# moxime/joint-vae

Hardware: AMD Instinct MI355X
Metric: training_images_per_sec (higher is better)
Workload: dtype f32

## Files before the change

### include/jvae_hip.h

```cpp
#ifndef JVAE_HIP_H
#define JVAE_HIP_H

#include <stddef.h>

#ifdef __cplusplus
extern "C" {
#endif

const char* jvae_version(void);

int jvae_gemm_f32(int M, int N, int K, int batch,
                  const float* A, long sAm, long sAk, long sAb,
                  const float* B, long sBk, long sBn, long sBb,
                  float* C, long sCm, long sCn, long sCb,
                  const float* bias, int bias_mode, int flags, int splitk, void* stream);

int jvae_splitk_fold_f32(const float* part, const float* bias, float* y, int S, long MN, int N, int relu, int accumulate,
                         void* stream);

size_t jvae_conv2d_workspace_bytes(int N, int Cin, int H, int W, int Cout, int KH, int KW, int S, int P, int OP,
                                   int transposed);
int jvae_conv2d_set_split_bf16(int mode);
int jvae_conv2d_set_split_shape16(int on);
int jvae_conv2d_out_shape(int H, int W, int KH, int KW, int S, int P, int OP, int transposed, int* OH, int* OW);
int jvae_conv2d_route(int dir, int layout, int bias, int stats, int y_f32, int aff_kind,
                      int N, int Cin, int H, int W, int Cout, int KH, int KW, int S, int P, int OP, int transposed,
                      int* kernel, int* swap, size_t* ws_bytes, int* splits, int* aff_ok);
const char* jvae_conv2d_kernel_name(int kernel);
int jvae_conv2d_fwd_f32(const float* x, const float* w, const float* bias, float* y,
                        int N, int Cin, int H, int W, int Cout, int KH, int KW, int S, int P, int OP, int transposed,
                        void* ws, size_t ws_bytes, void* stream);
int jvae_conv2d_stats_splits(int N, int Cin, int H, int W, int Cout, int KH, int KW, int S, int P, int OP, int transposed);
int jvae_conv2d_fwd_stats_f32(const float* x, const float* w, const float* bias, float* y, float* stats, int* nsplit,
                              int N, int Cin, int H, int W, int Cout, int KH, int KW, int S, int P, int OP, int transposed,
                              void* ws, size_t ws_bytes, void* stream);
int jvae_conv2d_dgrad_f32(const float* dy, const float* w, float* dx,
                          int N, int Cin, int H, int W, int Cout, int KH, int KW, int S, int P, int OP, int transposed,
                          void* ws, size_t ws_bytes, void* stream);
int jvae_conv2d_wgrad_f32(const float* x, const float* dy, float* dw, float* dbias, int accumulate,
                          int N, int Cin, int H, int W, int Cout, int KH, int KW, int S, int P, int OP, int transposed,
                          void* ws, size_t ws_bytes, void* stream);

int jvae_pack_cache_configure(void* buf, size_t bytes);
int jvae_pack_cache_begin(void* stream, long long owner, const void* const* weights, int n);
int jvae_pack_cache_end(void);
int jvae_pack_cache_pin(void);
int jvae_pack_cache_reset(void);
int jvae_pack_cache_stats(int* entries, long long* hits, long long* misses, long long* refreshes);

size_t jvae_channel_sum_workspace_bytes(int C);
int jvae_channel_sum_f32(const float* t, float* out, int N, int C, int P, int accumulate, void* ws, size_t ws_bytes,
                         void* stream);

size_t jvae_bn_workspace_bytes(int C);
int jvae_bn_plan(int N, int C, int P, int* nsplit, int* nchunk);
int jvae_image_range(int N, int parts, int j, int* nb, int* ne);
// ... 295 lines not shown
```

### joint-vae_amd/csrc/conv_api.hip

```cpp
#include "common.h"
#include "jvae_internal.h"
#include "conv_dispatch.h"

namespace {

inline ConvRoute route(const ConvGeom& g, int transposed, ConvDir dir, CallFlags f = {}) {
    return jvae_conv_route(g, transposed, dir, CONV_F32, f);
}

bool affine_ok(const ConvGeom& g, int transposed, ConvDir other, const ConvRoute& r) {
    return r.aff_ok && route(g, transposed, other, {false, false, false, 1}).aff_ok;
}

int fwd_f32(const float* x, const float* w, const float* bias, float* y, float* stats, int* nsplit, const InAff* aff,
            int N, int Cin, int H, int W, int Cout, int KH, int KW, int S, int P, int OP, int transposed,
            void* ws, size_t ws_bytes, void* stream) {
    ConvGeom g; int oh, ow;
    if (nsplit) *nsplit = 0;
    if (!jvae_make_geom(N, Cin, H, W, Cout, KH, KW, S, P, OP, transposed, &g, &oh, &ow)) return JVAE_EINVAL;
    const ConvRoute r = route(g, transposed, CONV_FWD, {bias != nullptr, stats != nullptr, false, jvae_aff_kind(aff)});
    if (aff && !affine_ok(g, transposed, CONV_WGRAD, r)) return JVAE_ENOTSUP;
    if (N == 0) return 0;
    if (jvae_ws_short(r, ws, ws_bytes)) return JVAE_EWORKSPACE;
    return jvae_conv_run_fwd(r, g, x, w, bias, y, (float*)ws, ws_bytes, (hipStream_t)stream, stats, nsplit, aff);
// ... 39 lines not shown
    if (!jvae_make_geom(N, Cin, H, W, Cout, KH, KW, S, P, OP, transposed, &g, &oh, &ow)) return 0;
    return jvae_conv_ws(g, transposed);
}

int jvae_conv2d_route(int dir, int layout, int bias, int stats, int y_f32, int aff_kind,
                      int N, int Cin, int H, int W, int Cout, int KH, int KW, int S, int P, int OP, int transposed,
                      int* kernel, int* swap, size_t* ws_bytes, int* splits, int* aff_ok) {
    ConvGeom g; int oh, ow;
    if (dir != CONV_FWD && dir != CONV_DGRAD && dir != CONV_WGRAD) return JVAE_EINVAL;
    if ((layout != CONV_F32 && layout != CONV_B8) || aff_kind < 0 || aff_kind > 2) return JVAE_EINVAL;
    if (!jvae_make_geom(N, Cin, H, W, Cout, KH, KW, S, P, OP, transposed, &g, &oh, &ow)) return JVAE_EINVAL;
    const ConvRoute r = jvae_conv_route(g, transposed, (ConvDir)dir, (ConvLayout)layout,
                                        {bias != 0, stats != 0, y_f32 != 0, aff_kind});
    if (kernel) *kernel = (int)r.k;
    if (swap) *swap = r.swap ? 1 : 0;
    if (ws_bytes) *ws_bytes = r.ws;
    if (splits) *splits = r.splits;
    if (aff_ok) *aff_ok = r.aff_ok ? 1 : 0;
    return 0;
}

const char* jvae_conv2d_kernel_name(int kernel) {
    switch (kernel) {
#define JVAE_CK_NAME(k) case k: return #k;
        JVAE_CK_NAME(CK_NONE) JVAE_CK_NAME(CK_GENERIC) JVAE_CK_NAME(CK_POINT) JVAE_CK_NAME(CK_SMALLCO)
        JVAE_CK_NAME(CK_SMALLCI) JVAE_CK_NAME(CK_FWD5) JVAE_CK_NAME(CK_FWD5_X3) JVAE_CK_NAME(CK_T2) JVAE_CK_NAME(CK_T2_X3)
        JVAE_CK_NAME(CK_WG5) JVAE_CK_NAME(CK_WG5_X3) JVAE_CK_NAME(CK_B8) JVAE_CK_NAME(CK_T2_B8) JVAE_CK_NAME(CK_WG_B8)
        JVAE_CK_NAME(CK_WG_B8X) JVAE_CK_NAME(CK_SMALLCO_DG)
#undef JVAE_CK_NAME
        default: return nullptr;
    }
}

int jvae_conv2d_out_shape(int H, int W, int KH, int KW, int S, int P, int OP, int transposed, int* OH, int* OW) {
    ConvGeom g;
    if (!OH || !OW) return JVAE_EINVAL;
    return jvae_make_geom(1, 1, H, W, 1, KH, KW, S, P, OP, transposed, &g, OH, OW) ? 0 : JVAE_EINVAL;
}

int jvae_conv2d_fwd_f32(const float* x, const float* w, const float* bias, float* y,
                        int N, int Cin, int H, int W, int Cout, int KH, int KW, int S, int P, int OP, int transposed,
                        void* ws, size_t ws_bytes, void* stream) {
    if (!w || (N > 0 && (!x || !y))) return JVAE_EINVAL;
    return fwd_f32(x, w, bias, y, nullptr, nullptr, nullptr, N, Cin, H, W, Cout, KH, KW, S, P, OP, transposed, ws, ws_bytes,
                   stream);
}

int jvae_conv2d_stats_splits(int N, int Cin, int H, int W, int Cout, int KH, int KW, int S, int P, int OP, int transposed) {
    ConvGeom g; int oh, ow;
    if (!jvae_make_geom(N, Cin, H, W, Cout, KH, KW, S, P, OP, transposed, &g, &oh, &ow)) return 0;
    return route(g, transposed, CONV_FWD, {false, true, false, 0}).splits;
}

int jvae_conv2d_fwd_stats_f32(const float* x, const float* w, const float* bias, float* y, float* stats, int* nsplit,
                              int N, int Cin, int H, int W, int Cout, int KH, int KW, int S, int P, int OP, int transposed,
                              void* ws, size_t ws_bytes, void* stream) {
    if (!w || !nsplit || (N > 0 && (!x || !y))) return JVAE_EINVAL;
    return fwd_f32(x, w, bias, y, stats, nsplit, nullptr, N, Cin, H, W, Cout, KH, KW, S, P, OP, transposed, ws, ws_bytes, stream);
}

int jvae_conv2d_affine_ok(int N, int Cin, int H, int W, int Cout, int KH, int KW, int S, int P, int OP, int transposed) {
    ConvGeom g; int oh, ow;
    if (!jvae_make_geom(N, Cin, H, W, Cout, KH, KW, S, P, OP, transposed, &g, &oh, &ow)) return 0;
    return affine_ok(g, transposed, CONV_WGRAD, route(g, transposed, CONV_FWD, {false, false, false, 1})) ? 1 : 0;
}

// ... 47 lines not shown
```

### joint-vae_amd/csrc/conv_dispatch.h

```cpp
#pragma once
#include "common.h"
#include "jvae_internal.h"

size_t jvae_conv_generic_ws(const ConvGeom& g);
int jvae_fold_fwd(const ConvGeom& g, const float* xb, const float* w, const float* bias, float* ys,
                  float* ws, size_t ws_bytes, hipStream_t st);
int jvae_fold_bwd(const ConvGeom& g, const float* ys, const float* w, const float* bias, float* xb,
                  float* ws, size_t ws_bytes, hipStream_t st);
int jvae_fold_wgrad(const ConvGeom& g, const float* xb, const float* ys, float* dw,
                    float* ws, size_t ws_bytes, hipStream_t st);
size_t jvae_channel_sum_ws_bytes(int C);
int jvae_channel_sum(const float* t, float* out, int N, int C, int P, int accumulate, float* ws, size_t ws_bytes,
                     hipStream_t st);

bool jvae_conv5_fwd_ok(int Cin, int H, int W, int Cout, int OH, int OW, int S, int P);
size_t jvae_conv5_pack_floats(int Cin, int Cout);
int jvae_conv5_fwd(const float* in, const float* w, int swap, int flip, const float* bias, float* out,
                   int N, int Cin, int H, int W, int Cout, int OW, int S, int P, float* ws, hipStream_t st,
                   float* stats = nullptr, int* nsplit = nullptr, const InAff* aff = nullptr);
int jvae_conv5_fwd_max_splits(int N, int OW);

int jvae_conv5_pack(const float* w, float* wp, int C, int O, int swap, int flip, hipStream_t st);

bool jvae_conv5_x3_ok(int Cin, int H, int W, int Cout, int OH, int OW, int S, int P);
// ... 3 lines not shown
bool jvae_conv5_x3_enabled();
int jvae_conv5_x3_wpack(const float* w, float* ws, int C, int O, int swap, int flip, hipStream_t st);
bool jvae_convt2_x3_ok(int N, int C, int WS, int O);
int jvae_convt2_x3(const float* in, const float* w, const float* bias, float* out, int N, int C, int WS, int O, float* ws,
                   hipStream_t st, float* stats = nullptr, int* nsplit = nullptr, const InAff* aff = nullptr);
int jvae_conv5_x3_fwd(const float* in, const float* w, int swap, int flip, const float* bias, float* out,
                      int N, int Cin, int H, int W, int Cout, int OW, int S, int P, float* ws, hipStream_t st,
                      float* stats = nullptr, int* nsplit = nullptr, const InAff* aff = nullptr);

bool jvae_convt2_ok(int C, int HS, int WS, int O, int HB, int WB, int KH, int KW, int S, int P);
int jvae_convt2(const float* in, const float* wpacked, const float* bias, float* out, int N, int C, int WS, int O,
                hipStream_t st, float* stats = nullptr, int* nsplit = nullptr, const InAff* aff = nullptr);

bool jvae_conv5_smallco_ok(int Cin, int H, int W, int Cout, int KH, int KW, int S, int P);
int jvae_conv5_smallco(const float* in, const float* w, const float* bias, float* out, int N, int Cin, int W, int Cout,
                       hipStream_t st, const InAff* aff = nullptr);
int jvae_conv5_smallco_dgrad(const float* dy, const float* w, float* dx, int N, int Cy, int W, int Cx, hipStream_t st);

bool jvae_conv5_smallci_ok(int Cin, int H, int W, int Cout, int OW, int S, int P, bool dgrad_role);
int jvae_conv5_smallci(const float* in, const float* w, int swap, int flip, const float* bias, float* out,
                       int N, int Cin, int W, int Cout, float* ws, hipStream_t st, float* stats = nullptr, int* nsplit = nullptr);

bool jvae_conv5_wgrad_ok(int Ca, int HS, int WS, int Cb, int HB, int WB, int S, int P);
size_t jvae_conv5_wgrad_ws_floats(int N, int Ca, int Cb, int S, int WS);
int jvae_conv5_wgrad(const float* ps, const float* q, float* dw, int accumulate, int swapflip,
                     int N, int Ca, int WS, int Cb, int S, int P, float* ws, hipStream_t st,
                     const InAff* aff_p = nullptr, const InAff* aff_q = nullptr);

bool jvae_conv5_wgrad_x3_ok(int Ca, int HS, int WS, int Cb, int HB, int WB, int S, int P);
size_t jvae_conv5_wgrad_x3_ws_floats(int N, int Ca, int Cb, int S);
int jvae_conv5_wgrad_x3(const float* ps, const float* q, float* dw, int accumulate, int swapflip,
                        int N, int Ca, int WS, int Cb, int S, int P, float* ws, hipStream_t st,
                        const InAff* aff_p = nullptr, const InAff* aff_q = nullptr);

bool jvae_make_geom(int N, int Cin, int H, int W, int Cout, int KH, int KW, int S, int P, int OP, int transposed,
                    ConvGeom* g, int* OH, int* OW);

enum ConvDir { CONV_FWD = 1, CONV_DGRAD = 2, CONV_WGRAD = 4 };
enum ConvLayout { CONV_F32, CONV_B8 };
enum ConvKernel {
    CK_NONE,
    CK_GENERIC, CK_POINT,
    CK_SMALLCO, CK_SMALLCI, CK_FWD5, CK_FWD5_X3, CK_T2, CK_T2_X3, CK_WG5, CK_WG5_X3,
    CK_B8, CK_T2_B8, CK_WG_B8, CK_WG_B8X,
    CK_SMALLCO_DG,
};
struct CallFlags {
    bool bias, stats;
    bool y_f32;
    int aff;
};
struct ConvRoute {
    ConvKernel k;
    bool swap;
    int S, P;
    size_t ws;
    int splits;
    bool aff_ok;
};
ConvRoute jvae_conv_route(const ConvGeom& g, int transposed, ConvDir dir, ConvLayout layout, CallFlags f);
inline int jvae_aff_kind(const InAff* aff) { return !aff ? 0 : (aff->relu == JVAE_ACT_LEAKY ? 2 : 1); }
inline bool jvae_ws_short(const ConvRoute& r, const void* ws, size_t ws_bytes) { return r.ws && (!ws || ws_bytes < r.ws); }
template <class T>
inline void jvae_wgrad_operands(const ConvRoute& r, int transposed, T* x, T* dy, const InAff* aff, T** ps, T** q,
                                const InAff** aff_p, const InAff** aff_q) {
    const bool p_is_x = r.swap != (transposed != 0);
    *ps = p_is_x ? x : dy;
    *q = p_is_x ? dy : x;
    *aff_p = p_is_x ? aff : nullptr;
    *aff_q = p_is_x ? nullptr : aff;
}

size_t jvae_conv_ws(const ConvGeom& g, int transposed);
int jvae_conv_run_fwd(const ConvRoute& r, const ConvGeom& g, const float* in, const float* w, const float* bias, float* out,
                      float* ws, size_t ws_bytes, hipStream_t st, float* stats = nullptr, int* nsplit = nullptr,
                      const InAff* aff = nullptr);
int jvae_conv_run_wgrad(const ConvRoute& r, const ConvGeom& g, int transposed, const float* x, const float* dy, float* dw,
                        float* ws, size_t ws_bytes, hipStream_t st, const InAff* aff = nullptr);
```

### joint-vae_amd/csrc/conv_dispatch.hip

```cpp
#include "common.h"
#include "conv_dispatch.h"
#include "conv_b8.h"
#include "pack_elems.h"

namespace {

inline bool is5(const ConvGeom& g) { return g.KH == 5 && g.KW == 5; }
inline bool is3p1(const ConvGeom& g) { return g.KH == 3 && g.KW == 3 && g.P == 1; }
inline size_t max_sz(size_t a, size_t b) { return a > b ? a : b; }

inline bool point_input(const ConvGeom& g) {
    return g.Hs == 1 && g.Ws == 1 && g.P == 0 && g.S == 1 && g.Hb == g.KH && g.Wb == g.KW;
}
inline int point_wgrad_pieces(const ConvGeom& g) {
    const int want = (int)(1024 / ((long)cdiv(g.Cs, 64) * cdiv(g.Cb * g.KH * g.KW, 64)));
    return want < 1 ? 1 : (want > 8 ? 8 : want);
}

struct FwdOp { int Ci, H, W, Co, OH, OW; };
inline FwdOp fwd_op(const ConvGeom& g, bool small_in) {
    return small_in ? FwdOp{g.Cs, g.Hs, g.Ws, g.Cb, g.Hb, g.Wb} : FwdOp{g.Cb, g.Hb, g.Wb, g.Cs, g.Hs, g.Ws};
}
struct WgOp { int Ca, HS, WS, Cb, HB, WB; };
inline WgOp wg_op(const ConvGeom& g, bool swap) {
// ... 73 lines not shown
}

inline const float* packed_f32(const float* w, float* ws, int C, int O, int swap, int flip, hipStream_t st) {
    return (const float*)jvae_packed(JVAE_PACK_F32, w, C, O, swap, flip, ws,
                                     [&](void* dst) { return jvae_conv5_pack(w, (float*)dst, C, O, swap, flip, st); });
}

}

bool jvae_make_geom(int N, int Cin, int H, int W, int Cout, int KH, int KW, int S, int P, int OP, int transposed,
                    ConvGeom* g, int* OH, int* OW) {
    if (N < 0 || Cin <= 0 || Cout <= 0 || H <= 0 || W <= 0 || KH <= 0 || KW <= 0 || S <= 0 || P < 0 || OP < 0)
        return false;
    g->N = N; g->KH = KH; g->KW = KW; g->S = S; g->P = P;
    if (!transposed) {
        if (OP != 0) return false;
        *OH = (H + 2 * P - KH) / S + 1;
        *OW = (W + 2 * P - KW) / S + 1;
        g->Cb = Cin; g->Hb = H; g->Wb = W;
        g->Cs = Cout; g->Hs = *OH; g->Ws = *OW;
    } else {
        if (OP >= S && OP != 0) return false;
        *OH = (H - 1) * S - 2 * P + KH + OP;
        *OW = (W - 1) * S - 2 * P + KW + OP;
        g->Cs = Cin; g->Hs = H; g->Ws = W;
        g->Cb = Cout; g->Hb = *OH; g->Wb = *OW;
    }
    return *OH > 0 && *OW > 0;
}

ConvRoute jvae_conv_route(const ConvGeom& g, int transposed, ConvDir dir, ConvLayout layout, CallFlags f) {
    if (dir == CONV_WGRAD) return wgrad_route(g, transposed, layout == CONV_B8, f);
    return fwd_route(g, transposed, dir, layout == CONV_B8, f);
}

size_t jvae_conv_ws(const ConvGeom& g, int transposed) {
    size_t a = max_sz(jvae_conv_generic_ws(g), jvae_channel_sum_ws_bytes(g.Cb > g.Cs ? g.Cb : g.Cs));
    for (ConvDir d : {CONV_FWD, CONV_DGRAD, CONV_WGRAD}) a = max_sz(a, jvae_conv_route(g, transposed, d, CONV_F32, {}).ws);
    if (is5(g)) a = max_sz(a, 4 * jvae_conv5_pack_floats(g.Cb, g.Cs));
    if (transposed && point_input(g)) a = max_sz(a, 4 * (size_t)8 * g.Cs * g.Cb * g.KH * g.KW);
    return a;
}

int jvae_conv_run_fwd(const ConvRoute& r, const ConvGeom& g, const float* in, const float* w, const float* bias, float* out,
                      float* ws, size_t ws_bytes, hipStream_t st, float* stats, int* nsplit, const InAff* aff) {
    const FwdOp o = fwd_op(g, r.swap);
    const int sw = r.swap ? 1 : 0;
    switch (r.k) {
        case CK_SMALLCO: return jvae_conv5_smallco(in, w, bias, out, g.N, g.Cb, g.Wb, g.Cs, st, aff);
        case CK_SMALLCO_DG: return jvae_conv5_smallco_dgrad(in, w, out, g.N, g.Cs, g.Wb, g.Cb, st);
        case CK_SMALLCI: return jvae_conv5_smallci(in, w, sw, sw, bias, out, g.N, o.Ci, o.W, o.Co, ws, st, stats, nsplit);
        case CK_FWD5_X3:
            return jvae_conv5_x3_fwd(in, w, sw, sw, bias, out, g.N, o.Ci, o.H, o.W, o.Co, o.OW, r.S, r.P, ws, st, stats, nsplit, aff);
        case CK_FWD5:
            return jvae_conv5_fwd(in, w, sw, sw, bias, out, g.N, o.Ci, o.H, o.W, o.Co, o.OW, r.S, r.P, ws, st, stats, nsplit, aff);
        case CK_T2_X3: return jvae_convt2_x3(in, w, bias, out, g.N, g.Cs, g.Ws, g.Cb, ws, st, stats, nsplit, aff);
        case CK_T2: {
            const float* wp = packed_f32(w, ws, g.Cs, g.Cb, 1, 0, st);
            if (!wp) return JVAE_EINVAL;
            return jvae_convt2(in, wp, bias, out, g.N, g.Cs, g.Ws, g.Cb, st, stats, nsplit, aff);
        }
        case CK_POINT: {
            const int cols = g.Cb * g.KH * g.KW;
            if (r.swap)
                return jvae_gemm_launch_ex(g.N, cols, g.Cs, 1, in, g.Cs, 1, 0, w, cols, 1, 0, out, cols, 1, 0,
                                           bias, bias ? 1 : 0, g.KH * g.KW, 0, 1, st);
// ... 41 lines not shown
```

### joint-vae_amd/csrc/conv_wgrad_x3.hip

```cpp
#include <stdlib.h>
#include "common.h"
#include "jvae_internal.h"
#include "conv_dispatch.h"
#include "conv_x3.h"

namespace {

typedef x3_bf16x8 bf16x8;
typedef __bf16 bf16x4 __attribute__((ext_vector_type(4)));
typedef x3_u32x4 u32x4;
typedef x3_f32x2 f32x2;
typedef __attribute__((address_space(3))) bf16x4 lds_bf16x4;

struct WgX3P {
    const void* ps;
    const void* q;
    float* slab;
    int N, Ca, Cb, P, G;
    InAff aff_p, aff_q;
};

template <int S, int WS, int MODE, int NPL = 3>
struct WgX3Geom {
    static constexpr int HS = WS;
// ... 437 lines not shown
                else if (MODE == 2) { b = cbq0 * 8 + c16; tap = wave + 4 * (2 * t + cb); }
                else if (MODE == 3) { b = j & 3; tap = tile * 8 + (j >> 2); }
                else { b = j & 7; tap = tile * 4 + (j >> 3); }
                if (b >= p.Cb || tap > 24) continue;
#pragma unroll
                for (int rb = 0; rb < 2; ++rb)
#pragma unroll
                    for (int r = 0; r < 4; ++r) {
                        const int a = a0 + rb * 16 + g16 * 4 + r;
                        if (a < p.Ca) slab[((long)a * 25 + tap) * p.Cb + b] = acc16[t][rb][cb][r];
                    }
            }
        }
        return;
    }
#pragma unroll
    for (int t = 0; t < G::NBT; ++t) {
        const int tile = wave + 4 * t;
        if (tile >= G::NTILE) continue;
        int b, tap;
        if (MODE == 0) { b = cbq0 * 8 + l31; tap = tile; }
        else if (MODE == 2) { b = cbq0 * 8 + (l31 & 15); tap = tile * 2 + (l31 >> 4); }
        else if (MODE == 3) { b = l31 & 3; tap = tile * 8 + (l31 >> 2); }
        else { b = l31 & 7; tap = tile * 4 + (l31 >> 3); }
        if (b >= p.Cb || tap > 24) continue;
#pragma unroll
        for (int r = 0; r < 16; ++r) {
            const int a = a0 + (r & 3) + 8 * (r >> 2) + 4 * half;
            if (a < p.Ca) slab[((long)a * 25 + tap) * p.Cb + b] = acc[t][r];
        }
    }
}

template <int S, int WS, int MODE, int NPL = 3>
int launch_wgx3(const WgX3P& p, hipStream_t st) {
    using G = WgX3Geom<S, WS, MODE, NPL>;
    static_assert(G::LDS_BYTES + 2048 <= 80 * 1024, "two workgroups per CU must fit the 160 KB LDS");
    dim3 grid(p.G, (p.Ca + 31) / 32, (p.Cb + 8 * G::NCBQ - 1) / (8 * G::NCBQ));
    if (MODE == 1 || MODE == 3) grid.z = 1;
    const bool aff = p.aff_p.sc || p.aff_q.sc;
    const bool leaky = (p.aff_p.sc && p.aff_p.relu == JVAE_ACT_LEAKY) || (p.aff_q.sc && p.aff_q.relu == JVAE_ACT_LEAKY);
    if constexpr (NPL == 1) {
        static bool attr1 = false;
        if (!attr1) {
            const void* fns[2] = {reinterpret_cast<const void*>(&conv5_wgrad_x3_kernel<S, WS, MODE, 0, true, 1>),
                                  reinterpret_cast<const void*>(&conv5_wgrad_x3_kernel<S, WS, MODE, 1, true, 1>)};
            for (const void* f : fns) {
                hipError_t e = hipFuncSetAttribute(f, hipFuncAttributeMaxDynamicSharedMemorySize, G::LDS_BYTES);
                if (e != hipSuccess) return (int)e;
            }
            attr1 = true;
        }
        if (aff) hipLaunchKernelGGL((conv5_wgrad_x3_kernel<S, WS, MODE, 1, true, 1>), grid, dim3(256), G::LDS_BYTES, st, p);
        else hipLaunchKernelGGL((conv5_wgrad_x3_kernel<S, WS, MODE, 0, true, 1>), grid, dim3(256), G::LDS_BYTES, st, p);
        JVAE_LAUNCH_CHECK();
        return 0;
    } else {
    static bool attr_set = false;
    auto kernel = [](auto A) { return &conv5_wgrad_x3_kernel<S, WS, MODE, decltype(A)::value, true>; };
    if (const int rc = jvae_aff_lds_attr(attr_set, G::LDS_BYTES, kernel)) return rc;
    jvae_with_aff(leaky ? 2 : (aff ? 1 : 0), [&](auto A) { hipLaunchKernelGGL(kernel(A), grid, dim3(256), G::LDS_BYTES, st, p); });
    JVAE_LAUNCH_CHECK();
    return 0;
    }
}

inline int x3_mode(int S, int Cb) { return Cb <= 4 ? 3 : (Cb <= 8 ? 1 : (S == 2 ? 2 : 0)); }

int slab_count_x3(int N, int Ca, int Cb, int S) {
    const int mode = x3_mode(S, Cb);
    const int gz = (mode == 1 || mode == 3) ? 1 : (mode == 2 ? (Cb + 15) / 16 : (Cb + 31) / 32);
    const int per = ((Ca + 31) / 32) * gz;
    int target = 512 / per;
    if (target < 1) target = 1;
    int imgs = (N + target - 1) / target;
    if (imgs < 1) imgs = 1;
    return (N + imgs - 1) / imgs;
}

}

bool jvae_conv5_wgrad_x3_ok(int Ca, int HS, int WS, int Cb, int HB, int WB, int S, int P) {
    if (!jvae_conv5_x3_enabled()) return false;
    if (S != 1 && S != 2) return false;
    if (HS != WS || HB != WB || WB != WS * S) return false;
    if (WS != 8 && WS != 16 && WS != 32) return false;
    if (P < 0 || P > 4 || Ca < 16 || Cb < 1) return false;
    if (P + WB > (WS - 1) * S + 5) return false;
    return true;
}

size_t jvae_conv5_wgrad_x3_ws_floats(int N, int Ca, int Cb, int S) { return (size_t)slab_count_x3(N, Ca, Cb, S) * Ca * Cb * 25; }

int jvae_conv5_wgrad_x3(const float* ps, const float* q, float* dw, int accumulate, int swapflip,
                        int N, int Ca, int WS, int Cb, int S, int P, float* ws, hipStream_t st,
                        const InAff* aff_p, const InAff* aff_q) {
    const InAff none{nullptr, nullptr, 0};
    WgX3P p{ps, q, ws, N, Ca, Cb, P, slab_count_x3(N, Ca, Cb, S), aff_p ? *aff_p : none, aff_q ? *aff_q : none};
    int rc = JVAE_ENOTSUP;
    const int mode = x3_mode(S, Cb);
#define WGX3_CASE(S_, WS_, M_) case WS_: rc = launch_wgx3<S_, WS_, M_>(p, st); break;
    if (mode == 3 && S == 1) {
        switch (WS) { WGX3_CASE(1, 8, 3) WGX3_CASE(1, 16, 3) WGX3_CASE(1, 32, 3) }
    } else if (mode == 3) {
        switch (WS) { WGX3_CASE(2, 8, 3) WGX3_CASE(2, 16, 3) WGX3_CASE(2, 32, 3) }
    } else if (mode == 1 && S == 1) {
        switch (WS) { WGX3_CASE(1, 8, 1) WGX3_CASE(1, 16, 1) WGX3_CASE(1, 32, 1) }
    } else if (mode == 1) {
        switch (WS) { WGX3_CASE(2, 8, 1) WGX3_CASE(2, 16, 1) WGX3_CASE(2, 32, 1) }
    } else if (mode == 0) {
        switch (WS) { WGX3_CASE(1, 8, 0) WGX3_CASE(1, 16, 0) WGX3_CASE(1, 32, 0) }
    } else {
        switch (WS) { WGX3_CASE(2, 8, 2) WGX3_CASE(2, 16, 2) WGX3_CASE(2, 32, 2) }
    }
#undef WGX3_CASE
    if (rc) return rc;
    return jvae_wgrad_slab_reduce(ws, dw, p.G, Ca, Cb, accumulate, swapflip, st, 1);
}

bool jvae_conv5_wgrad_b8x_ok(int Ca, int HS, int WS, int Cb, int HB, int WB, int S, int P) {
    if (S != 1 && S != 2) return false;
    if (HS != WS || HB != WB || WB != WS * S) return false;
    if (WS != 8 && WS != 16 && WS != 32 && !(WS == 64 && S == 1)) return false;
    if (P < 0 || P > 4 || Ca < 16 || Cb < 1) return false;
    if (P + WB > (WS - 1) * S + 5) return false;
    return true;
}

size_t jvae_conv5_wgrad_b8x_ws_floats(int N, int Ca, int Cb, int S) { return (size_t)slab_count_x3(N, Ca, Cb, S) * Ca * Cb * 25; }

int jvae_conv5_wgrad_b8x(const void* ps, const void* q, float* dw, int accumulate, int swapflip,
                         int N, int Ca, int WS, int Cb, int S, int P, float* ws, hipStream_t st,
                         const InAff* aff_p, const InAff* aff_q) {
    const InAff none{nullptr, nullptr, 0};
    WgX3P p{ps, q, ws, N, Ca, Cb, P, slab_count_x3(N, Ca, Cb, S), aff_p ? *aff_p : none, aff_q ? *aff_q : none};
// ... 21 lines not shown
```

### joint-vae_amd/jvae_hip/lib.py

```python
import ctypes
import os
from ctypes import c_char_p, c_float, c_int, c_long, c_longlong, c_size_t, c_void_p, POINTER

import torch

_HERE = os.path.dirname(os.path.abspath(__file__))
LIB_PATH = os.environ.get('JVAE_HIP_LIB') or os.path.join(_HERE, 'libjvae_hip.so')

_lib = None

P = c_void_p
_SIGS = {
    'jvae_version': (c_char_p, []),
    'jvae_gemm_f32': (c_int, [c_int] * 4 + [P, c_long, c_long, c_long] * 3 + [P, c_int, c_int, c_int, P]),
    'jvae_splitk_fold_f32': (c_int, [P, P, P, c_int, c_long, c_int, c_int, c_int, P]),
    'jvae_conv2d_workspace_bytes': (c_size_t, [c_int] * 11),
    'jvae_conv2d_set_split_bf16': (c_int, [c_int]),
    'jvae_conv2d_set_split_shape16': (c_int, [c_int]),
    'jvae_conv2d_out_shape': (c_int, [c_int] * 8 + [POINTER(c_int), POINTER(c_int)]),
    'jvae_conv2d_route': (c_int, [c_int] * 17 + [POINTER(c_int), POINTER(c_int), POINTER(c_size_t), POINTER(c_int), POINTER(c_int)]),
    'jvae_conv2d_kernel_name': (c_char_p, [c_int]),
    'jvae_conv2d_fwd_f32': (c_int, [P, P, P, P] + [c_int] * 11 + [P, c_size_t, P]),
    'jvae_conv2d_stats_splits': (c_int, [c_int] * 11),
    'jvae_conv2d_fwd_stats_f32': (c_int, [P, P, P, P, P, POINTER(c_int)] + [c_int] * 11 + [P, c_size_t, P]),
    'jvae_conv2d_dgrad_f32': (c_int, [P, P, P] + [c_int] * 11 + [P, c_size_t, P]),
    'jvae_conv2d_wgrad_f32': (c_int, [P, P, P, P, c_int] + [c_int] * 11 + [P, c_size_t, P]),
    'jvae_b8_pack_f32': (c_int, [P, P, c_int, c_int, c_long, P]),
    'jvae_b8_unpack_f32': (c_int, [P, P, c_int, c_int, c_long, c_int, P]),
    'jvae_conv2d_native_b8': (c_int, [c_int] * 11),
    'jvae_conv2d_workspace_bytes_b8': (c_size_t, [c_int] * 11),
    'jvae_conv2d_stats_splits_b8': (c_int, [c_int] * 11),
    'jvae_conv2d_fwd_b8': (c_int, [P, P, P, P, c_int, P, POINTER(c_int)] + [c_int] * 11 + [P, c_size_t, P]),
    'jvae_conv2d_dgrad_b8': (c_int, [P, P, P] + [c_int] * 11 + [P, c_size_t, P]),
    'jvae_conv2d_wgrad_b8': (c_int, [P, P, P, P, c_int] + [c_int] * 11 + [P, c_size_t, P]),
    'jvae_bn_workspace_bytes_b8': (c_size_t, [c_int]),
    'jvae_bn_plan_b8': (c_int, [c_int, c_int, c_long, POINTER(c_int), POINTER(c_int)]),
    'jvae_bn_fwd_b8': (c_int, [P] * 9 + [c_int, c_int, c_long, c_float, c_float, c_int, c_int, P, c_int, P, P, c_size_t, P]),
    'jvae_bn_bwd_b8': (c_int, [P] * 9 + [c_int, c_int, c_int, c_long, c_int, P, c_size_t, P]),
    'jvae_bn_finalize_b8': (c_int, [P] * 9 + [c_int, c_int, c_long, c_float, c_float, c_int, P, c_int, P, P, c_size_t, P]),
    'jvae_bn_sums_b8': (c_int, [P, P, P, c_int, c_int, c_long, P, c_size_t, P]),
    'jvae_bn_fwd_sync_b8': (c_int, [P] * 9 + [c_int, c_int, c_long, c_float, c_float, c_int, P, P, c_int, P, c_size_t, P]),
    'jvae_bn_bwd_sums_b8': (c_int, [P] * 7 + [c_int, c_int, c_long, c_int, P, c_size_t, P]),
    'jvae_bn_bwd_sync_b8': (c_int, [P] * 8 + [c_int, P, P, P, c_int, c_int, c_int, c_long, c_int, P, c_size_t, P]),
    'jvae_conv2d_affine_ok_b8': (c_int, [c_int] * 11),
    'jvae_conv2d_fwd_aff_b8': (c_int, [P, P, P, P, c_int, P, POINTER(c_int), P, P, c_int] + [c_int] * 11 + [P, c_size_t, P]),
    'jvae_conv2d_wgrad_aff_b8': (c_int, [P, P, P, P, c_int, P, P, c_int] + [c_int] * 11 + [P, c_size_t, P]),
    'jvae_relu_fwd_b8': (c_int, [P, P, c_long, P]),
    'jvae_relu_bwd_b8': (c_int, [P, P, P, c_long, P]),
    'jvae_bn_finalize_f32': (c_int, [P] * 10 + [c_int, c_int, c_int, c_float, c_float, c_int, P, c_int, P, P, c_size_t, P]),
    'jvae_conv2d_affine_ok': (c_int, [c_int] * 11),
    'jvae_conv2d_fwd_aff_f32': (c_int, [P, P, P, P, P, POINTER(c_int), P, P, c_int] + [c_int] * 11 + [P, c_size_t, P]),
# ... 216 lines not shown
```

### joint-vae_amd/jvae_hip/ops.py

```python
import collections
import contextlib
import ctypes
import math
from ctypes import byref, c_int, c_size_t

import numpy as np
import torch

from . import lib as L

RELU, SIGMOID, IDENT, LEAKY = 1, 2, 0, 3
BN_ACT = {IDENT: 0, RELU: 1, LEAKY: 2}
OVERLAP_WGRAD = True
ACT_KIND = {'relu': RELU, 'sigmoid': SIGMOID, 'linear': IDENT, 'leaky': LEAKY, None: IDENT}


def _c(t):
    return t if t.is_contiguous() else t.contiguous()


def _f32(t, what):
    if t.dtype != torch.float32:
        raise L.JvaeHipError(f'{what}: fp32 expected, got {t.dtype}')
    return t
# ... 169 lines not shown
    lib = L.load()
    N, _, H, W = x.shape
    geom = spec.geom(N, H, W)
    cap = _geom_query('jvae_conv2d_stats_splits', geom)
    if cap <= 0:
        return conv_fwd_raw(x, w, b, spec), None, 0
    oh, ow = spec.out_hw(H, W)
    y = torch.empty((N, spec.cout, oh, ow), device=x.device, dtype=torch.float32)
    stats = torch.empty((spec.cout * cap * 2,), device=x.device, dtype=torch.float32)
    ws, nb = _conv_ws(geom, x.device)
    ns = c_int(0)
    rc = lib.jvae_conv2d_fwd_stats_f32(L.ptr(x), L.ptr(w), L.ptr(b), L.ptr(y), L.ptr(stats), byref(ns), *geom,
                                       L.ptr(ws), nb, L.stream_ptr())
    L.check(rc, 'jvae_conv2d_fwd_stats_f32')
    return y, (stats if ns.value > 0 else None), ns.value


def conv_affine_ok(spec, N, H, W):
    return bool(_geom_query('jvae_conv2d_affine_ok', spec.geom(N, H, W)))


ConvRoute = collections.namedtuple('ConvRoute', 'kernel swap ws splits aff_ok')
ROUTE_DIR = {'fwd': 1, 'dgrad': 2, 'wgrad': 4}
ROUTE_LAYOUT = {'f32': 0, 'b8': 1}


def conv_route(spec, N, H, W, direction, layout='f32', bias=False, stats=False, y_f32=False, aff=0):
    lib = L.load()
    k, sw, ns, ok, ws = c_int(), c_int(), c_int(), c_int(), c_size_t()
    rc = lib.jvae_conv2d_route(ROUTE_DIR[direction], ROUTE_LAYOUT[layout], int(bias), int(stats), int(y_f32), int(aff),
                               *spec.geom(N, H, W), byref(k), byref(sw), byref(ws), byref(ns), byref(ok))
    L.check(rc, 'jvae_conv2d_route')
    return ConvRoute(lib.jvae_conv2d_kernel_name(k.value).decode(), bool(sw.value), ws.value, ns.value, bool(ok.value))


class LaunchProbe:

    def __init__(self, match):
        self.match, self.events, self.armed = match, [], False

    def times_ms(self):
        return [a.elapsed_time(b) for a, b in self.events]


FWD_AFF_PROBE = None


def conv_fwd_aff_raw(x, w, b, spec, aff, want_stats):
    lib = L.load()
    N, _, H, W = x.shape
    geom = spec.geom(N, H, W)
    oh, ow = spec.out_hw(H, W)
    y = torch.empty((N, spec.cout, oh, ow), device=x.device, dtype=torch.float32)
    stats, ns = None, c_int(0)
    if want_stats:
        cap = _geom_query('jvae_conv2d_stats_splits', geom)
        if cap > 0:
            stats = torch.empty((spec.cout * cap * 2,), device=x.device, dtype=torch.float32)
    ws, nb = _conv_ws(geom, x.device)
    probe = FWD_AFF_PROBE
    timed = probe is not None and probe.armed and probe.match(spec, N, H)
    if timed:
        ev = (torch.cuda.Event(enable_timing=True), torch.cuda.Event(enable_timing=True))
        ev[0].record()
    rc = lib.jvae_conv2d_fwd_aff_f32(L.ptr(x), L.ptr(w), L.ptr(b), L.ptr(y), L.ptr(stats), byref(ns),
                                     L.ptr(aff[0]), L.ptr(aff[1]), int(aff[2]), *geom, L.ptr(ws), nb, L.stream_ptr())
# ... 1691 lines not shown
```

Before: 144,000.

## Add K-packed bf16x3 MFMA weight-gradient kernel for 5x5 stride-1 small-Cb convs

Adds a new wgrad kernel for 5x5 stride-1 convolutions with at most three output-side channels. It packs the kernel-width taps and channels into the MFMA K dimension using shifted LDS copies of the q rows, instead of using the mode-3 layout that wastes MFMA lanes. Global loads for the next tile are overlapped with the MFMA loop, and the kernel is enabled by default through an env toggle. The cost is a more complex LDS layout, extra MFMAs on two waves to cover the fifth kernel row, and higher LDS use per workgroup.

```diff
diff --git a/include/jvae_hip.h b/include/jvae_hip.h
--- a/include/jvae_hip.h
+++ b/include/jvae_hip.h
@@ -22,6 +22,8 @@
                                    int transposed);
 int jvae_conv2d_set_split_bf16(int mode);
 int jvae_conv2d_set_split_shape16(int on);
+int jvae_conv2d_set_wgrad_kpack(int on);
+const char* jvae_conv2d_wgrad_form(int N, int Cin, int H, int W, int Cout, int KH, int KW, int S, int P, int OP, int transposed);
 int jvae_conv2d_out_shape(int H, int W, int KH, int KW, int S, int P, int OP, int transposed, int* OH, int* OW);
 int jvae_conv2d_route(int dir, int layout, int bias, int stats, int y_f32, int aff_kind,
                       int N, int Cin, int H, int W, int Cout, int KH, int KW, int S, int P, int OP, int transposed,
diff --git a/joint-vae_amd/csrc/conv_api.hip b/joint-vae_amd/csrc/conv_api.hip
--- a/joint-vae_amd/csrc/conv_api.hip
+++ b/joint-vae_amd/csrc/conv_api.hip
@@ -95,6 +95,14 @@
     }
 }
 
+int jvae_conv2d_set_wgrad_kpack(int on) { return jvae_conv5_wgrad_x3_set_kpack(on); }
+
+const char* jvae_conv2d_wgrad_form(int N, int Cin, int H, int W, int Cout, int KH, int KW, int S, int P, int OP, int transposed) {
+    ConvGeom g; int oh, ow;
+    if (!jvae_make_geom(N, Cin, H, W, Cout, KH, KW, S, P, OP, transposed, &g, &oh, &ow)) return nullptr;
+    return jvae_conv_wgrad_form(g, transposed);
+}
+
 int jvae_conv2d_out_shape(int H, int W, int KH, int KW, int S, int P, int OP, int transposed, int* OH, int* OW) {
     ConvGeom g;
     if (!OH || !OW) return JVAE_EINVAL;
diff --git a/joint-vae_amd/csrc/conv_dispatch.h b/joint-vae_amd/csrc/conv_dispatch.h
--- a/joint-vae_amd/csrc/conv_dispatch.h
+++ b/joint-vae_amd/csrc/conv_dispatch.h
@@ -59,6 +59,8 @@
 int jvae_conv5_wgrad_x3(const float* ps, const float* q, float* dw, int accumulate, int swapflip,
                         int N, int Ca, int WS, int Cb, int S, int P, float* ws, hipStream_t st,
                         const InAff* aff_p = nullptr, const InAff* aff_q = nullptr);
+int jvae_conv5_wgrad_x3_set_kpack(int on);
+const char* jvae_conv5_wgrad_x3_form(int Cb, int S);
 
 bool jvae_make_geom(int N, int Cin, int H, int W, int Cout, int KH, int KW, int S, int P, int OP, int transposed,
                     ConvGeom* g, int* OH, int* OW);
@@ -86,6 +88,7 @@
     bool aff_ok;
 };
 ConvRoute jvae_conv_route(const ConvGeom& g, int transposed, ConvDir dir, ConvLayout layout, CallFlags f);
+const char* jvae_conv_wgrad_form(const ConvGeom& g, int transposed);
 inline int jvae_aff_kind(const InAff* aff) { return !aff ? 0 : (aff->relu == JVAE_ACT_LEAKY ? 2 : 1); }
 inline bool jvae_ws_short(const ConvRoute& r, const void* ws, size_t ws_bytes) { return r.ws && (!ws || ws_bytes < r.ws); }
 template <class T>
diff --git a/joint-vae_amd/csrc/conv_dispatch.hip b/joint-vae_amd/csrc/conv_dispatch.hip
--- a/joint-vae_amd/csrc/conv_dispatch.hip
+++ b/joint-vae_amd/csrc/conv_dispatch.hip
@@ -129,6 +129,12 @@
 ConvRoute jvae_conv_route(const ConvGeom& g, int transposed, ConvDir dir, ConvLayout layout, CallFlags f) {
     if (dir == CONV_WGRAD) return wgrad_route(g, transposed, layout == CONV_B8, f);
     return fwd_route(g, transposed, dir, layout == CONV_B8, f);
+}
+
+const char* jvae_conv_wgrad_form(const ConvGeom& g, int transposed) {
+    const ConvRoute r = wgrad_route(g, transposed, false, {});
+    if (r.k != CK_WG5_X3) return "";
+    return jvae_conv5_wgrad_x3_form(wg_op(g, r.swap).Cb, r.S);
 }
 
 size_t jvae_conv_ws(const ConvGeom& g, int transposed) {
diff --git a/joint-vae_amd/csrc/conv_wgrad_x3.hip b/joint-vae_amd/csrc/conv_wgrad_x3.hip
--- a/joint-vae_amd/csrc/conv_wgrad_x3.hip
+++ b/joint-vae_amd/csrc/conv_wgrad_x3.hip
@@ -493,6 +493,286 @@
     }
 }
 
+template <int WS>
+struct WgKpGeom {
+    static constexpr int TPIX = WS >= 16 ? 128 : 64;
+    static constexpr int TH = TPIX / WS;
+    static constexpr int TILES = WS * WS / TPIX;
+    static constexpr int ROWS = TH + 4;
+    static constexpr int NG = (WS + 8) / 4;
+    static constexpr int RPE = 4 * NG;
+    static constexpr int CB = 3;
+    static constexpr int REGS = (ROWS * RPE * 2 + 127) / 128 * 128;
+    static constexpr int QPL = 4 * CB * REGS + 128;
+    __host__ __device__ static constexpr int region(int r) { return r * REGS + (r < 3 ? 16 * r : 8 * (r + 3)); }
+    static constexpr int RW = 64 / NG;
+    static_assert(4 * RW >= CB * ROWS, "the four waves cover the patch rows of the three channels");
+    static constexpr int PS = 4 * TPIX;
+    static constexpr int PITEMS = 4 * (TPIX / 2);
+    static constexpr int LDS_BYTES = 3 * (QPL + PS * 16);
+    static_assert(QPL % 16 == 0 && (RPE * 2) % 8 == 0, "aligned planes and rows");
+};
+
+typedef unsigned int u32x2 __attribute__((ext_vector_type(2)));
+
+__device__ __forceinline__ bf16x8 lds_pix8(const unsigned char* base, int off) {
+    const bf16x4 lo = *(const lds_bf16x4*)(base + off);
+    const bf16x4 hi = *(const lds_bf16x4*)(base + off + 8);
+    return __builtin_shufflevector(lo, hi, 0, 1, 2, 3, 4, 5, 6, 7);
+}
+
+template <int WS, int AFF>
+__global__ __launch_bounds__(256, 2) void conv5_wgrad_x3_kpack_kernel(WgX3P p) {
+    using G = WgKpGeom<WS>;
+    extern __shared__ __attribute__((aligned(16))) unsigned char lds_raw[];
+    unsigned char* const Qw = lds_raw;
+    u32x4* const Pt = reinterpret_cast<u32x4*>(lds_raw + 3 * G::QPL);
+    const unsigned char* const Qb = lds_raw;
+    const unsigned char* const Pb = lds_raw + 3 * G::QPL;
+    constexpr int NT8 = 8;
+    __shared__ __attribute__((aligned(16))) float ctab[AFF ? 2 * NT8 : 4];
+
+    const int tid = threadIdx.x, lane = tid & 63, wave = tid >> 6;
+    const int a0 = blockIdx.y * 32;
+    if (AFF && tid < NT8) {
+        const bool ok = p.aff_q.sc && tid < p.Cb;
+        ctab[tid] = ok ? p.aff_q.sc[tid] : 0.f;
+        ctab[NT8 + tid] = ok ? p.aff_q.sh[tid] : 0.f;
+    }
+    float cr[16];
+    if constexpr (AFF != 0) {
+        const int ch0 = a0 + (tid % 4) * 8;
+#pragma unroll
+        for (int ci = 0; ci < 8; ++ci) {
+            const bool ok = p.aff_p.sc && ch0 + ci < p.Ca;
+            cr[ci] = ok ? p.aff_p.sc[ch0 + ci] : 0.f;
+            cr[8 + ci] = ok ? p.aff_p.sh[ch0 + ci] : 0.f;
+        }
+    }
+
+    const int g16 = lane >> 4, c16 = lane & 15, q4 = c16 >> 2, pp = lane & 3;
+    const int pl16 = 8 * g16 + q4;
+    const int aoff16 = (pl16 * 4 + (pp >> 1)) * 16 + (pp & 1) * 8;
+    const int kwc = c16 / 3 > 4 ? 4 : c16 / 3, cc = c16 == 15 ? 0 : c16 % 3;
+    const int lp = 8 * g16;
+    const int bel = G::region((kwc & 3) * G::CB + cc) + ((lp / WS) * G::RPE + lp % WS + 4 * (kwc >> 2)) * 2;
+    const int boffw = bel + wave * G::RPE * 2;
+    const int boff4 = bel + 4 * G::RPE * 2;
+
+    f32x4 acc[2] = {f32x4{0.f, 0.f, 0.f, 0.f}, f32x4{0.f, 0.f, 0.f, 0.f}};
+    f32x4 accx = {0.f, 0.f, 0.f, 0.f};
+
+    const ImageRange ir = image_range(p.N, p.G, blockIdx.x);
+    constexpr int PU = (G::PITEMS + 255) / 256;
+    const long pcs = (long)WS * WS;
+    const int qrow = wave * G::RW + lane / G::NG, qm = lane % G::NG;
+    const bool qvalid = lane < G::RW * G::NG && qrow < G::CB * G::ROWS;
+    const int qc = qrow / G::ROWS, qlr = qrow % G::ROWS;
+    const bool qlive = qvalid && qc < p.Cb;
+    const int qcc = qvalid ? qc : 0;
+    float rq[4];
+    f32x2 rp[PU][8];
+    const float* const qf = (const float*)p.q;
+    const float* const psf = (const float*)p.ps;
+
+    auto gload = [&](int item) {
+        int tid = threadIdx.x;
+        asm volatile("" : "+v"(tid));
+        const int n = item / G::TILES, row0 = (item % G::TILES) * G::TH;
+        const int in_row0 = row0 - p.P;
+        {
+            const int irow = in_row0 + qlr, col0 = 4 * qm - p.P;
+            const bool ok = qlive && irow >= 0 && irow < WS;
+            const float* src = qf + (((long)n * p.Cb + qcc) * WS + (ok ? irow : 0)) * WS;
+#pragma unroll
+            for (int j = 0; j < 4; ++j) rq[j] = *((ok && (unsigned)(col0 + j) < (unsigned)WS) ? src + (col0 + j) : qf);
+        }
+#pragma unroll
+        for (int k = 0; k < PU; ++k) {
+            const int u = tid + k * 256;
+            const int c = u % 4, px2 = u / 4;
+            const int ch0 = a0 + c * 8;
+            const bool ok = u < G::PITEMS;
+            const float* src = psf + (((long)n * p.Ca + ch0) * WS + row0) * WS + 2 * px2;
+#pragma unroll
+            for (int ci = 0; ci < 8; ++ci)
+                rp[k][ci] = *reinterpret_cast<const f32x2*>((ok && ch0 + ci < p.Ca) ? src + ci * pcs : psf);
+        }
+    };
+    auto lstore = [&](int item) {
+        int tid = threadIdx.x;
+        asm volatile("" : "+v"(tid));
+        const int in_row0 = (item % G::TILES) * G::TH - p.P;
+        {
+            const int irow = in_row0 + qlr, col0 = 4 * qm - p.P;
+            const bool rowok = qlive && irow >= 0 && irow < WS;
+            const float sc = AFF ? ctab[qcc] : 0.f, sh = AFF ? ctab[NT8 + qcc] : 0.f;
+            float v[4];
+#pragma unroll
+            for (int j = 0; j < 4; ++j) {
+                const bool live = rowok && (unsigned)(col0 + j) < (unsigned)WS;
+                float x = rq[j];
+                if (AFF && p.aff_q.sc) {
+                    x = fmaf(x, sc, sh);
+                    if constexpr (AFF == 2) x = jvae_act(x, p.aff_q.relu);
+                    else if (p.aff_q.relu) x = fmaxf(x, 0.f);
+                }
+                v[j] = live ? x : 0.f;
+            }
+            unsigned w[3][2];
+            x3_split2(f32x2{v[0], v[1]}, w[0][0], w[1][0], w[2][0]);
+            x3_split2(f32x2{v[2], v[3]}, w[0][1], w[1][1], w[2][1]);
+            const bool last = qm == G::NG - 1;
+            unsigned char* dst = Qw + (qlr * G::RPE + 4 * qm) * 2;
+#pragma unroll
+            for (int plane = 0; plane < 3; ++plane) {
+                const unsigned a = w[plane][0], b = w[plane][1];
+                unsigned c = (unsigned)__shfl_down((int)a, 1), d = (unsigned)__shfl_down((int)b, 1);
+                c = last ? 0u : c; d = last ? 0u : d;
+                if (qvalid) {
+                    unsigned char* q0 = dst + plane * G::QPL;
+                    *reinterpret_cast<u32x2*>(q0 + G::region(0 * G::CB + qcc)) = u32x2{a, b};
+                    *reinterpret_cast<u32x2*>(q0 + G::region(1 * G::CB + qcc)) = u32x2{(a >> 16) | (b << 16), (b >> 16) | (c << 16)};
+                    *reinterpret_cast<u32x2*>(q0 + G::region(2 * G::CB + qcc)) = u32x2{b, c};
+                    *reinterpret_cast<u32x2*>(q0 + G::region(3 * G::CB + qcc)) = u32x2{(b >> 16) | (c << 16), (c >> 16) | (d << 16)};
+                }
+            }
+        }
+#pragma unroll
+        for (int k = 0; k < PU; ++k) {
+            const int u = tid + k * 256;
+            if (u < G::PITEMS) {
+                const int c = u % 4, px2 = u / 4;
+                const int nch = p.Ca - (a0 + c * 8);
+                const bool aff = p.aff_p.sc != nullptr;
+                const int relu = p.aff_p.relu;
+                f32x2 vv[8];
+#pragma unroll
+                for (int ci = 0; ci < 8; ++ci) {
+                    f32x2 v = ci < nch ? rp[k][ci] : f32x2{0.f, 0.f};
+                    if constexpr (AFF != 0) {
+                        if (aff) {
+                            f32x2 a{fmaf(v[0], cr[ci], cr[8 + ci]), fmaf(v[1], cr[ci], cr[8 + ci])};
+                            if constexpr (AFF == 2) { a[0] = jvae_act(a[0], relu); a[1] = jvae_act(a[1], relu); }
+                            else if (relu) { a[0] = fmaxf(a[0], 0.f); a[1] = fmaxf(a[1], 0.f); }
+                            v = ci < nch ? a : f32x2{0.f, 0.f};
+                        }
+                    }
+                    vv[ci] = v;
+                }
+                u32x4 sp[2][3];
+#pragma unroll
+                for (int cp = 0; cp < 4; ++cp)
+#pragma unroll
+                    for (int j = 0; j < 2; ++j) {
+                        unsigned hh, mm, ll;
+                        x3_split2(f32x2{vv[2 * cp][j], vv[2 * cp + 1][j]}, hh, mm, ll);
+                        sp[j][0][cp] = hh; sp[j][1][cp] = mm; sp[j][2][cp] = ll;
+                    }
+#pragma unroll
+                for (int plane = 0; plane < 3; ++plane) {
+                    Pt[plane * G::PS + (2 * px2) * 4 + c] = sp[0][plane];
+                    Pt[plane * G::PS + (2 * px2 + 1) * 4 + c] = sp[1][plane];
+                }
+            }
+        }
+    };
+
+    constexpr int KS = G::TPIX / 32;
+    constexpr int APL[6] = {0, 2, 1, 0, 1, 0}, BPL[6] = {2, 0, 1, 1, 0, 0};
+    auto read_a = [&](int ks, bf16x8 (&d)[2][3]) {
+#pragma unroll
+        for (int rb = 0; rb < 2; ++rb)
+#pragma unroll
+            for (int plane = 0; plane < 3; ++plane)
+                d[rb][plane] = tr_pair<256>(Pb + plane * G::PS * 16, aoff16 + rb * 32 + ks * 32 * 64);
+    };
+    auto read_b = [&](int ks, int off, bf16x8 (&d)[3]) {
+        const int koff = (ks * 32 / WS) * G::RPE * 2;
+#pragma unroll
+        for (int plane = 0; plane < 3; ++plane) d[plane] = lds_pix8(Qb + plane * G::QPL, off + koff);
+    };
+
+    const int item_beg = ir.nb * G::TILES, item_end = ir.ne * G::TILES;
+    if (item_beg < item_end) gload(item_beg);
+    for (int item = item_beg; item < item_end; ++item) {
+        __syncthreads();
+        lstore(item);
+        __syncthreads();
+        bf16x8 a[2][2][3], b[2][3], bx[2][3];
+        read_a(0, a[0]);
+        read_b(0, boffw, b[0]);
+        read_b(0, boff4, bx[0]);
+        __builtin_amdgcn_sched_barrier(0);
+        if (item + 1 < item_end) gload(item + 1);
+        __builtin_amdgcn_sched_barrier(0);
+#pragma unroll
+        for (int ks = 0; ks < KS; ++ks) {
+            const int cur = ks & 1;
+            if (ks + 1 < KS) {
+                read_a(ks + 1, a[cur ^ 1]);
+                read_b(ks + 1, boffw, b[cur ^ 1]);
+                read_b(ks + 1, boff4, bx[cur ^ 1]);
+            }
+            __builtin_amdgcn_sched_barrier(0);
+#pragma unroll
+            for (int m = 0; m < 6; ++m)
+#pragma unroll
+                for (int rb = 0; rb < 2; ++rb)
+                    acc[rb] = __builtin_amdgcn_mfma_f32_16x16x32_bf16(a[cur][rb][APL[m]], b[cur][BPL[m]], acc[rb], 0, 0, 0);
+            if (wave < 2) {
+                bf16x8 aq[3];
+#pragma unroll
+                for (int plane = 0; plane < 3; ++plane) {
+                    const u32x4 x1 = __builtin_bit_cast(u32x4, a[cur][1][plane]), x0 = __builtin_bit_cast(u32x4, a[cur][0][plane]);
+                    u32x4 xs;
+#pragma unroll
+                    for (int e = 0; e < 4; ++e) xs[e] = (wave & 1) ? x1[e] : x0[e];
+                    aq[plane] = __builtin_bit_cast(bf16x8, xs);
+                }
+#pragma unroll
+                for (int m = 0; m < 6; ++m)
+                    accx = __builtin_amdgcn_mfma_f32_16x16x32_bf16(aq[APL[m]], bx[cur][BPL[m]], accx, 0, 0, 0);
+            }
+            __builtin_amdgcn_sched_barrier(0);
+        }
+    }
+
+    float* slab = p.slab + (long)blockIdx.x * p.Ca * (p.Cb * 25);
+    const int kw = c16 / 3, cb = c16 % 3;
+    if (kw < 5 && cb < p.Cb) {
+#pragma unroll
+        for (int rb = 0; rb < 2; ++rb)
+#pragma unroll
+            for (int r = 0; r < 4; ++r) {
+                const int a = a0 + rb * 16 + g16 * 4 + r;
+                if (a < p.Ca) slab[((long)a * 25 + wave * 5 + kw) * p.Cb + cb] = acc[rb][r];
+            }
+        if (wave < 2) {
+#pragma unroll
+            for (int r = 0; r < 4; ++r) {
+                const int a = a0 + wave * 16 + g16 * 4 + r;
+                if (a < p.Ca) slab[((long)a * 25 + 20 + kw) * p.Cb + cb] = accx[r];
+            }
+        }
+    }
+}
+
+template <int WS>
+int launch_wgkp(const WgX3P& p, hipStream_t st) {
+    using G = WgKpGeom<WS>;
+    static_assert(G::LDS_BYTES + 2048 <= 80 * 1024, "two workgroups per CU must fit the 160 KB LDS");
+    const dim3 grid(p.G, (p.Ca + 31) / 32, 1);
+    const bool aff = p.aff_p.sc || p.aff_q.sc;
+    const bool leaky = (p.aff_p.sc && p.aff_p.relu == JVAE_ACT_LEAKY) || (p.aff_q.sc && p.aff_q.relu == JVAE_ACT_LEAKY);
+    static bool attr_set = false;
+    auto kernel = [](auto A) { return &conv5_wgrad_x3_kpack_kernel<WS, decltype(A)::value>; };
+    if (const int rc = jvae_aff_lds_attr(attr_set, G::LDS_BYTES, kernel)) return rc;
+    jvae_with_aff(leaky ? 2 : (aff ? 1 : 0), [&](auto A) { hipLaunchKernelGGL(kernel(A), grid, dim3(256), G::LDS_BYTES, st, p); });
+    JVAE_LAUNCH_CHECK();
+    return 0;
+}
+
 template <int S, int WS, int MODE, int NPL = 3>
 int launch_wgx3(const WgX3P& p, hipStream_t st) {
     using G = WgX3Geom<S, WS, MODE, NPL>;
@@ -528,6 +808,9 @@
 
 inline int x3_mode(int S, int Cb) { return Cb <= 4 ? 3 : (Cb <= 8 ? 1 : (S == 2 ? 2 : 0)); }
 
+int g_kpack = [] { const char* e = getenv("JVAE_WGRAD_KPACK"); return (e && e[0] == '0') ? 0 : 1; }();
+inline bool x3_kpack(int S, int Cb) { return g_kpack && S == 1 && Cb <= 3; }
+
 int slab_count_x3(int N, int Ca, int Cb, int S) {
     const int mode = x3_mode(S, Cb);
     const int gz = (mode == 1 || mode == 3) ? 1 : (mode == 2 ? (Cb + 15) / 16 : (Cb + 31) / 32);
@@ -553,6 +836,22 @@
 
 size_t jvae_conv5_wgrad_x3_ws_floats(int N, int Ca, int Cb, int S) { return (size_t)slab_count_x3(N, Ca, Cb, S) * Ca * Cb * 25; }
 
+int jvae_conv5_wgrad_x3_set_kpack(int on) {
+    const int old = g_kpack;
+    g_kpack = on ? 1 : 0;
+    return old;
+}
+
+const char* jvae_conv5_wgrad_x3_form(int Cb, int S) {
+    if (x3_kpack(S, Cb)) return "kpack";
+    switch (x3_mode(S, Cb)) {
+        case 0: return "mode0";
+        case 1: return "mode1";
+        case 2: return "mode2";
+        default: return "mode3";
+    }
+}
+
 int jvae_conv5_wgrad_x3(const float* ps, const float* q, float* dw, int accumulate, int swapflip,
                         int N, int Ca, int WS, int Cb, int S, int P, float* ws, hipStream_t st,
                         const InAff* aff_p, const InAff* aff_q) {
@@ -561,7 +860,13 @@
     int rc = JVAE_ENOTSUP;
     const int mode = x3_mode(S, Cb);
 #define WGX3_CASE(S_, WS_, M_) case WS_: rc = launch_wgx3<S_, WS_, M_>(p, st); break;
-    if (mode == 3 && S == 1) {
+    if (x3_kpack(S, Cb)) {
+        switch (WS) {
+            case 8: rc = launch_wgkp<8>(p, st); break;
+            case 16: rc = launch_wgkp<16>(p, st); break;
+            case 32: rc = launch_wgkp<32>(p, st); break;
+        }
+    } else if (mode == 3 && S == 1) {
         switch (WS) { WGX3_CASE(1, 8, 3) WGX3_CASE(1, 16, 3) WGX3_CASE(1, 32, 3) }
     } else if (mode == 3) {
         switch (WS) { WGX3_CASE(2, 8, 3) WGX3_CASE(2, 16, 3) WGX3_CASE(2, 32, 3) }
diff --git a/joint-vae_amd/jvae_hip/lib.py b/joint-vae_amd/jvae_hip/lib.py
--- a/joint-vae_amd/jvae_hip/lib.py
+++ b/joint-vae_amd/jvae_hip/lib.py
@@ -17,6 +17,8 @@
     'jvae_conv2d_workspace_bytes': (c_size_t, [c_int] * 11),
     'jvae_conv2d_set_split_bf16': (c_int, [c_int]),
     'jvae_conv2d_set_split_shape16': (c_int, [c_int]),
+    'jvae_conv2d_set_wgrad_kpack': (c_int, [c_int]),
+    'jvae_conv2d_wgrad_form': (c_char_p, [c_int] * 11),
     'jvae_conv2d_out_shape': (c_int, [c_int] * 8 + [POINTER(c_int), POINTER(c_int)]),
     'jvae_conv2d_route': (c_int, [c_int] * 17 + [POINTER(c_int), POINTER(c_int), POINTER(c_size_t), POINTER(c_int), POINTER(c_int)]),
     'jvae_conv2d_kernel_name': (c_char_p, [c_int]),
diff --git a/joint-vae_amd/jvae_hip/ops.py b/joint-vae_amd/jvae_hip/ops.py
--- a/joint-vae_amd/jvae_hip/ops.py
+++ b/joint-vae_amd/jvae_hip/ops.py
@@ -225,6 +225,13 @@
                                *spec.geom(N, H, W), byref(k), byref(sw), byref(ws), byref(ns), byref(ok))
     L.check(rc, 'jvae_conv2d_route')
     return ConvRoute(lib.jvae_conv2d_kernel_name(k.value).decode(), bool(sw.value), ws.value, ns.value, bool(ok.value))
+
+
+def conv_wgrad_form(spec, N, H, W):
+    r = L.load().jvae_conv2d_wgrad_form(*spec.geom(N, H, W))
+    if r is None:
+        raise L.JvaeHipError('jvae_conv2d_wgrad_form: invalid geometry')
+    return r.decode()
 
 
 class LaunchProbe:
```

Measured after the change: 144,200 (median of 3 runs). Within noise of the previous version (+0.1%).
